# underdoc-wang/MPGCN

Measured on NVIDIA H100. Metric: OD-cells/sec (B*T*N^2), MPGCN hot path fwd+bwd, higher is better.
Workload: dtype f16

## Files before the change

mpgcn_b200/csrc/tc_engine.cuh:

```cuda
#pragma once

#include "common.cuh"
#include "wgmma.cuh"

#include <type_traits>

namespace mpgcn {
namespace tc {

enum AKind : int { A_MN128 = 0, A_K128 = 1, A_K64 = 2, A_MN64 = 3 };

struct OperandMap {
  int z_div, z_mod, z_mul;
  int seg_mod, seg_mul, seg_hi_mul;
  int k_seg;
};

struct Epilogue {
  void* out;
  __half* out16;
  long long sZ, sI, sR;
  int m_valid, r_valid;
  int out_f16;
  int relu;
  const float* bias;
  float alpha;
  const float* alpha_dev;
  float* absmax_out;
  const __half* corr_src;
  const float* corr_delta;
  long long cZ, cI, cR, cSeg;
  int corr_nseg;
};

struct alignas(64) GemmParams {
  CUtensorMap a_map;
  CUtensorMap b_map;
  OperandMap am, bm;
  int MT, NT, Z;
  int R;
  int kb_total, kb_per_seg;
  int split_k, kb_per_slice;
  int stages;
  int b_res_reps;
  int z_inner;
  Epilogue ep;
};

constexpr int kConsumerWGs = 2;
constexpr int kThreads1 = 128 * kConsumerWGs;
constexpr int kEpiRow = 40;
constexpr size_t kEpiBytes = (size_t)kConsumerWGs * 2 * 64 * kEpiRow * sizeof(float);

template <int AK, int BK>
struct Cfg {
  static constexpr int A_STAGE = (AK == A_MN128) ? BK * 256 : (AK == A_K128) ? 128 * 128 : (AK == A_K64) ? 128 * 64 * (BK / 32) : 4 * BK * 64;
  static constexpr bool A_MN = (AK == A_MN128) || (AK == A_MN64);
  static constexpr uint32_t A_KSTEP = (AK == A_MN128) ? 16 * 128 : (AK == A_MN64) ? 16 * 64 : 32;
  static constexpr uint32_t A_LBO = (AK == A_MN128) ? BK * 128 : (AK == A_MN64) ? BK * 64 : 16;
  static constexpr uint32_t A_SBO = (AK == A_MN128 || AK == A_K128) ? 1024 : 512;
  static constexpr uint32_t A_LAYOUT = (AK == A_MN128 || AK == A_K128) ? GMMA_SW128 : GMMA_SW64;
  static constexpr uint32_t B_KSTEP = 16 * 64;
  static constexpr uint32_t B_LBO = BK * 64;
  static constexpr uint32_t B_SBO = 512;
  static_assert(AK != A_K128 || BK == 64, "K-major SW128 rows hold exactly 64 halves");
  static_assert(AK != A_K64 || BK % 32 == 0, "K-major SW64 rows hold exactly 32 halves: BK counts whole planes");
  static constexpr uint32_t A_WG = (AK == A_MN128) ? BK * 128 : (AK == A_K128) ? 64 * 128 : (AK == A_K64) ? 64 * 64 : 2 * BK * 64;
  __host__ __device__ static constexpr uint32_t a_koff(int k) {
    return (AK == A_K64) ? (uint32_t)(k >> 1) * 8192u + (uint32_t)(k & 1) * 32u : (uint32_t)k * A_KSTEP;
  }
  static_assert(BK % 16 == 0, "wgmma K is 16 for fp16");
};

__host__ __device__ inline size_t smem_bytes(int a_stage, int R, int BK, int stages, int b_resident_tiles = 0) {
  const size_t b_stage = (size_t)R * BK * 64;
  return 1024  + (size_t)stages * a_stage + (size_t)(b_resident_tiles ? b_resident_tiles : stages) * b_stage + kEpiBytes +
         512 ;
}

#ifdef __CUDACC__
__device__ __forceinline__ void decode_tile(const GemmParams& p, int t, int& mt, int& nt, int& z) {
  if (p.z_inner > 1) {
    mt = t % p.MT;
    int rest = t / p.MT;
    const int zi = rest % p.z_inner;
    rest /= p.z_inner;
    nt = rest % p.NT;
    z = (rest / p.NT) * p.z_inner + zi;
  } else {
    mt = t % p.MT;
    const int rest = t / p.MT;
    nt = rest % p.NT;
    z = rest / p.NT;
  }
}

__device__ __forceinline__ void st_global_256(void* ptr, uint32_t a0, uint32_t a1, uint32_t a2, uint32_t a3, uint32_t a4, uint32_t a5,
                                              uint32_t a6, uint32_t a7) {
  uint4* d = reinterpret_cast<uint4*>(ptr);
  d[0] = make_uint4(a0, a1, a2, a3);
  d[1] = make_uint4(a4, a5, a6, a7);
}
__device__ __forceinline__ uint32_t pack_h2(float a, float b) { return f2h2_sat_bits(a, b); }

__device__ __forceinline__ void store_chunk(const Epilogue& ep, float alpha, const float* sbias, long long off,
                                            uint32_t (&acc)[32], float& amax) {
  float v[32];
#pragma unroll
  for (int c = 0; c < 32; ++c) {
    float x = __uint_as_float(acc[c]) * alpha;
    if (ep.bias) x += sbias[c];
    if (ep.relu) x = fmaxf(x, 0.f);
    v[c] = x;
  }
  if (ep.absmax_out) {
#pragma unroll
    for (int c = 0; c < 32; ++c) amax = fmaxf(amax, fabsf(v[c]));
  }
  if (ep.out_f16) {
    __half* dst = reinterpret_cast<__half*>(ep.out) + off;
#pragma unroll
    for (int q = 0; q < 2; ++q)
      st_global_256(dst + 16 * q, pack_h2(v[16 * q + 0], v[16 * q + 1]), pack_h2(v[16 * q + 2], v[16 * q + 3]),
                    pack_h2(v[16 * q + 4], v[16 * q + 5]), pack_h2(v[16 * q + 6], v[16 * q + 7]), pack_h2(v[16 * q + 8], v[16 * q + 9]),
                    pack_h2(v[16 * q + 10], v[16 * q + 11]), pack_h2(v[16 * q + 12], v[16 * q + 13]), pack_h2(v[16 * q + 14], v[16 * q + 15]));
  } else {
    float* dst = reinterpret_cast<float*>(ep.out) + off;
#pragma unroll
    for (int q = 0; q < 4; ++q)
      st_global_256(dst + 8 * q, __float_as_uint(v[8 * q + 0]), __float_as_uint(v[8 * q + 1]), __float_as_uint(v[8 * q + 2]),
                    __float_as_uint(v[8 * q + 3]), __float_as_uint(v[8 * q + 4]), __float_as_uint(v[8 * q + 5]),
                    __float_as_uint(v[8 * q + 6]), __float_as_uint(v[8 * q + 7]));
    if (ep.out16) {
      __half* d16 = ep.out16 + off;
#pragma unroll
      for (int q = 0; q < 2; ++q)
        st_global_256(d16 + 16 * q, pack_h2(v[16 * q + 0], v[16 * q + 1]), pack_h2(v[16 * q + 2], v[16 * q + 3]),
                      pack_h2(v[16 * q + 4], v[16 * q + 5]), pack_h2(v[16 * q + 6], v[16 * q + 7]), pack_h2(v[16 * q + 8], v[16 * q + 9]),
                      pack_h2(v[16 * q + 10], v[16 * q + 11]), pack_h2(v[16 * q + 12], v[16 * q + 13]), pack_h2(v[16 * q + 14], v[16 * q + 15]));
    }
  }
}

template <int AK, int BK>
__global__ void __launch_bounds__(kThreads1, 1) contract_kernel(const __grid_constant__ GemmParams p) {
  using C = Cfg<AK, BK>;
  constexpr int A_STAGE = C::A_STAGE;
  const int R = p.R;
  const int B_STAGE = R * BK * 64;
  const int S = p.stages;

  extern __shared__ uint8_t smem_raw[];
  uint8_t* smem = smem_raw + ((1024u - (smem_u32(smem_raw) & 1023u)) & 1023u);
  const int NRES = p.b_res_reps * p.kb_total;
  uint8_t* sA = smem;
  uint8_t* sB = sA + (size_t)S * A_STAGE;
  float* sEpi = reinterpret_cast<float*>(sB + (size_t)(NRES ? NRES : S) * B_STAGE);
  uint64_t* full = reinterpret_cast<uint64_t*>(reinterpret_cast<uint8_t*>(sEpi) + kEpiBytes);
  uint64_t* empty = full + S;
  uint64_t* bres_full = empty + S;
  float* sbias = reinterpret_cast<float*>(bres_full + 1);

  const int warp = threadIdx.x >> 5;
  const int lane = threadIdx.x & 31;

  if (threadIdx.x == 0) {
    tma_prefetch_desc(&p.a_map);
    tma_prefetch_desc(&p.b_map);
    for (int s = 0; s < S; ++s) {
      mbar_init(&full[s], 1);
      mbar_init(&empty[s], 4 * kConsumerWGs);
    }
    mbar_init(bres_full, 1);
    fence_barrier_init();
  }
  if (warp == 0) sbias[lane] = p.ep.bias ? p.ep.bias[lane] : 0.f;
  __syncthreads();

  const int num_tiles = p.MT * p.NT * p.Z;

  int p_t = blockIdx.x, p_kb = 0, p_kb1 = 0, p_kk = 0, p_sa_lo = 0, p_sa_hi = 0, p_sb_lo = 0, p_sb_hi = 0, p_zA0 = 0, p_zB0 = 0, p_mt = 0, p_nt = 0;
  int p_stage = 0;
  uint32_t p_phase = 0;
  auto p_start_tile = [&]() {
    int z;
    decode_tile(p, p_t, p_mt, p_nt, z);
    p_kb = p.split_k ? z * p.kb_per_slice : 0;
    p_kb1 = p.split_k ? min(p_kb + p.kb_per_slice, p.kb_total) : p.kb_total;
    p_zA0 = ((z / p.am.z_div) % p.am.z_mod) * p.am.z_mul;
    p_zB0 = ((z / p.bm.z_div) % p.bm.z_mod) * p.bm.z_mul;
    const int seg = p_kb / p.kb_per_seg;
    p_kk = p_kb - seg * p.kb_per_seg;
    p_sa_lo = seg % p.am.seg_mod; p_sa_hi = seg / p.am.seg_mod;
    p_sb_lo = seg % p.bm.seg_mod; p_sb_hi = seg / p.bm.seg_mod;
  };
  auto produce = [&]() {
    if (p_t >= num_tiles) return;
    mbar_wait_inline(&empty[p_stage], p_phase ^ 1u);
    mbar_arrive_expect_tx(&full[p_stage], (uint32_t)(A_STAGE + (NRES ? 0 : B_STAGE)));
    const int zA = p_zA0 + p_sa_lo * p.am.seg_mul + p_sa_hi * p.am.seg_hi_mul;
    const int zB = p_zB0 + p_sb_lo * p.bm.seg_mul + p_sb_hi * p.bm.seg_hi_mul;
    const int kA = p_kk * BK + p_sa_lo * p.am.k_seg;
    const int kB = p_kk * BK + p_sb_lo * p.bm.k_seg;
    uint8_t* a_dst = sA + (size_t)p_stage * A_STAGE;
    uint8_t* b_dst = sB + (size_t)p_stage * B_STAGE;
    if (AK == A_MN128) {
      tma_load_4d(a_dst, &p.a_map, &full[p_stage], p_mt * 128, kA, zA, 0);
      tma_load_4d(a_dst + BK * 128, &p.a_map, &full[p_stage], p_mt * 128 + 64, kA, zA, 0);
    } else if (AK == A_K128 || AK == A_K64) {
      tma_load_4d(a_dst, &p.a_map, &full[p_stage], kA, p_mt * 128, zA, 0);
    } else {
      tma_load_4d(a_dst, &p.a_map, &full[p_stage], 0, kA, p_mt * 4, zA);
    }
    if (!NRES)
      tma_load_4d(b_dst, &p.b_map, &full[p_stage], 0, kB, p_nt * R, zB);
    if (++p_stage == S) { p_stage = 0; p_phase ^= 1u; }
    if (++p_kk == p.kb_per_seg) {
      p_kk = 0;
      if (++p_sa_lo == p.am.seg_mod) { p_sa_lo = 0; ++p_sa_hi; }
      if (++p_sb_lo == p.bm.seg_mod) { p_sb_lo = 0; ++p_sb_hi; }
    }
    if (++p_kb == p_kb1) {
      p_t += gridDim.x;
      if (p_t < num_tiles) p_start_tile();
    }
  };
  if (threadIdx.x == 0 && (int)blockIdx.x < num_tiles) {
    if (NRES) {
      mbar_arrive_expect_tx(bres_full, (uint32_t)(NRES * B_STAGE));
      for (int sg = 0; sg < NRES; ++sg) {
        const int lo = sg % p.bm.seg_mod, hi = sg / p.bm.seg_mod;
        tma_load_4d(sB + (size_t)sg * B_STAGE, &p.b_map, bres_full, 0, lo * p.bm.k_seg, 0, lo * p.bm.seg_mul + hi * p.bm.seg_hi_mul);
      }
    }
    p_start_tile();
    for (int s = 0; s < S; ++s) produce();
  }
  __syncwarp();

  {
    const int wg = warp >> 2;
    const int tw = threadIdx.x & 127;
    const int wq = warp & 3, g = lane >> 2, q = lane & 3;
    const float alpha = p.ep.alpha_dev ? p.ep.alpha * __ldg(p.ep.alpha_dev) : p.ep.alpha;
    const uint64_t a_hi = gmma_desc_hi(C::A_SBO, C::A_LAYOUT);
    const uint64_t b_hi = gmma_desc_hi(C::B_SBO, GMMA_SW64);
    float* stg = sEpi + (size_t)wg * 2 * 64 * kEpiRow;
    float amax = 0.f;
    float acc[128];
    int stage = 0;
    uint32_t phase = 0;
    if (NRES && (int)blockIdx.x < num_tiles) mbar_wait_inline(bres_full, 0);
    for (int t = blockIdx.x; t < num_tiles; t += gridDim.x) {
      int mt, nt, z;
      decode_tile(p, t, mt, nt, z);
      const int kb0 = p.split_k ? z * p.kb_per_slice : 0;
      const int kb1 = p.split_k ? min(kb0 + p.kb_per_slice, p.kb_total) : p.kb_total;
      int prev = -1;
      for (int kb = kb0; kb < kb1; ++kb) {
        mbar_wait_inline(&full[stage], phase);
        const uint32_t a_addr = smem_u32(sA + (size_t)stage * A_STAGE) + C::A_WG * (uint32_t)wg;
        const int reps = NRES ? p.b_res_reps : 1;
        wgmma_fence();
        for (int rep = 0; rep < reps; ++rep) {
          const uint32_t b_addr = smem_u32(sB + (size_t)(NRES ? rep * p.kb_total + kb : stage) * B_STAGE);
          const int first = (kb == kb0 && rep == 0) ? 1 : 0;
          auto kblock = [&](auto width) {
            constexpr int RW = decltype(width)::value;
#pragma unroll
            for (int k = 0; k < BK / 16; ++k) {
              const uint64_t ad = gmma_desc(a_hi, a_addr + C::a_koff(k), C::A_LBO);
              const uint64_t bd = gmma_desc(b_hi, b_addr + k * C::B_KSTEP, C::B_LBO);
              wgmma_n<RW, C::A_MN ? 1 : 0, 1>(acc, ad, bd, (first && k == 0) ? 0 : 1);
            }
          };
          switch (R) {
            case 1: kblock(std::integral_constant<int, 1>()); break;
            case 2: kblock(std::integral_constant<int, 2>()); break;
            case 3: kblock(std::integral_constant<int, 3>()); break;
            case 4: kblock(std::integral_constant<int, 4>()); break;
            case 5: kblock(std::integral_constant<int, 5>()); break;
            case 6: kblock(std::integral_constant<int, 6>()); break;
            case 7: kblock(std::integral_constant<int, 7>()); break;
            default: kblock(std::integral_constant<int, 8>()); break;
          }
        }
        wgmma_commit();
        wgmma_wait<1>();
        if (prev >= 0) {
          __syncwarp();
          if (lane == 0) mbar_arrive(&empty[prev]);
          if (threadIdx.x == 0) produce();
          __syncwarp();
        }
        prev = stage;
        if (++stage == S) { stage = 0; phase ^= 1u; }
      }
      wgmma_wait<0>();
      if (prev >= 0) {
        __syncwarp();
        if (lane == 0) mbar_arrive(&empty[prev]);
        if (threadIdx.x == 0) produce();
        __syncwarp();
      }
      const int half = tw >> 6, rr = tw & 63;
      const int i = mt * 128 + wg * 64 + rr;
      const long long base = (long long)z * p.ep.sZ + (long long)i * p.ep.sI;
      float dl[8];
      long long cbase = 0;
      bool any_corr = false;
      if (p.ep.corr_src != nullptr) {
        const int zA = ((z / p.am.z_div) % p.am.z_mod) * p.am.z_mul;
        const int zB = ((z / p.bm.z_div) % p.bm.z_mod) * p.bm.z_mul;
        cbase = (long long)zB * p.ep.cZ + (long long)i * p.ep.cI;
#pragma unroll
        for (int sgi = 0; sgi < 8; ++sgi) {
          dl[sgi] = (sgi < p.ep.corr_nseg && i < p.ep.m_valid)
                        ? __ldg(p.ep.corr_delta + ((long long)zA * p.ep.corr_nseg + sgi) * p.ep.m_valid + i) : 0.f;
          any_corr |= (dl[sgi] != 0.f);
        }
      }
#pragma unroll
      for (int j0 = 0; j0 < 8; j0 += 2) {
        if (j0 < R) {
#pragma unroll
          for (int s = 0; s < 2; ++s) {
            if (j0 + s < R) {
#pragma unroll
              for (int jj = 0; jj < 4; ++jj)
#pragma unroll
                for (int h = 0; h < 2; ++h)
                  *reinterpret_cast<float2*>(stg + (s * 64 + 16 * wq + g + 8 * h) * kEpiRow + 8 * jj + 2 * q) =
                      make_float2(acc[16 * (j0 + s) + 4 * jj + 2 * h], acc[16 * (j0 + s) + 4 * jj + 2 * h + 1]);
            }
          }
          named_bar_sync(1 + wg, 128);
          const int j = j0 + half;
          const int r = nt * R + j;
          if (j < R && i < p.ep.m_valid && r < p.ep.r_valid) {
            uint32_t regs[32];
#pragma unroll
            for (int c = 0; c < 32; c += 4) {
              const float4 v = *reinterpret_cast<const float4*>(stg + (half * 64 + rr) * kEpiRow + c);
              regs[c] = __float_as_uint(v.x); regs[c + 1] = __float_as_uint(v.y);
              regs[c + 2] = __float_as_uint(v.z); regs[c + 3] = __float_as_uint(v.w);
            }
            if (any_corr) {
#pragma unroll
              for (int sgi = 0; sgi < 8; ++sgi) {
                if (sgi < p.ep.corr_nseg && dl[sgi] != 0.f) {
                  const uint4* src = reinterpret_cast<const uint4*>(p.ep.corr_src + cbase + (long long)sgi * p.ep.cSeg + (long long)r * p.ep.cR);
#pragma unroll
                  for (int qq = 0; qq < 4; ++qq) {
                    const uint4 v = __ldg(src + qq);
                    const __half2* h2 = reinterpret_cast<const __half2*>(&v);
#pragma unroll
                    for (int e = 0; e < 4; ++e) {
                      const float2 f = __half22float2(h2[e]);
                      regs[8 * qq + 2 * e] = __float_as_uint(fmaf(dl[sgi], f.x, __uint_as_float(regs[8 * qq + 2 * e])));
                      regs[8 * qq + 2 * e + 1] = __float_as_uint(fmaf(dl[sgi], f.y, __uint_as_float(regs[8 * qq + 2 * e + 1])));
                    }
                  }
                }
              }
            }
            store_chunk(p.ep, alpha, sbias, base + (long long)r * p.ep.sR, regs, amax);
          }
          named_bar_sync(1 + wg, 128);
        }
      }
    }
    if (p.ep.absmax_out) {
      for (int o = 16; o > 0; o >>= 1) amax = fmaxf(amax, __shfl_xor_sync(0xffffffffu, amax, o));
      if (lane == 0) atomicMax(reinterpret_cast<unsigned int*>(p.ep.absmax_out), __float_as_uint(amax));
    }
  }
}
#endif

int launch_contract(int ak, int bk, GemmParams& p, cudaStream_t stream);

}
}
```

Baseline: 392.9 million.

## Add dedicated TMA producer warpgroup with register reallocation to GEMM engine

Adds a third warpgroup that acts only as the TMA producer, giving up registers via setmaxnreg while the two consumer warpgroups raise their register budget. Consumers no longer issue produce() calls inline after each k-block, so loads for later tiles proceed without waiting on consumer progress. The correction-delta values are now re-read from global memory inside the epilogue instead of being held in an 8-entry register array, which lowers register pressure at the cost of extra loads. Waits switch to plain spin loops, and the launch now uses 384 threads per block, which lowers occupancy headroom.

Measured after the change: 398.8 million (median of 6 runs). 1.01x the previous value.

```diff
diff --git a/mpgcn_b200/csrc/tc_engine.cuh b/mpgcn_b200/csrc/tc_engine.cuh
--- a/mpgcn_b200/csrc/tc_engine.cuh
+++ b/mpgcn_b200/csrc/tc_engine.cuh
@@ -48,7 +48,9 @@
 };
 
 constexpr int kConsumerWGs = 2;
-constexpr int kThreads1 = 128 * kConsumerWGs;
+constexpr int kThreads1 = 128 * (1 + kConsumerWGs);
+constexpr int kProducerRegs = 40;
+constexpr int kConsumerRegs = 232;
 constexpr int kEpiRow = 40;
 constexpr size_t kEpiBytes = (size_t)kConsumerWGs * 2 * 64 * kEpiRow * sizeof(float);
 
@@ -102,6 +104,16 @@
   d[1] = make_uint4(a4, a5, a6, a7);
 }
 __device__ __forceinline__ uint32_t pack_h2(float a, float b) { return f2h2_sat_bits(a, b); }
+
+template <int REGS>
+__device__ __forceinline__ void setmaxnreg_dec() { asm volatile("setmaxnreg.dec.sync.aligned.u32 %0;" ::"n"(REGS)); }
+template <int REGS>
+__device__ __forceinline__ void setmaxnreg_inc() { asm volatile("setmaxnreg.inc.sync.aligned.u32 %0;" ::"n"(REGS)); }
+
+__device__ __forceinline__ void mbar_wait_spin(uint64_t* bar, uint32_t parity) {
+  while (!mbar_try_wait(bar, parity)) {
+  }
+}
 
 __device__ __forceinline__ void store_chunk(const Epilogue& ep, float alpha, const float* sbias, long long off,
                                             uint32_t (&acc)[32], float& amax) {
@@ -225,21 +237,29 @@
       if (p_t < num_tiles) p_start_tile();
     }
   };
-  if (threadIdx.x == 0 && (int)blockIdx.x < num_tiles) {
-    if (NRES) {
-      mbar_arrive_expect_tx(bres_full, (uint32_t)(NRES * B_STAGE));
-      for (int sg = 0; sg < NRES; ++sg) {
-        const int lo = sg % p.bm.seg_mod, hi = sg / p.bm.seg_mod;
-        tma_load_4d(sB + (size_t)sg * B_STAGE, &p.b_map, bres_full, 0, lo * p.bm.k_seg, 0, lo * p.bm.seg_mul + hi * p.bm.seg_hi_mul);
-      }
-    }
-    p_start_tile();
-    for (int s = 0; s < S; ++s) produce();
-  }
-  __syncwarp();
-
+  if (__shfl_sync(0xffffffffu, (int)threadIdx.x >> 7, 0) == 0) {
+    setmaxnreg_dec<kProducerRegs>();
+    if (threadIdx.x == 0 && (int)blockIdx.x < num_tiles) {
+      if (NRES) {
+        mbar_arrive_expect_tx(bres_full, (uint32_t)(NRES * B_STAGE));
+        for (int sg = 0; sg < NRES; ++sg) {
+          const int lo = sg % p.bm.seg_mod, hi = sg / p.bm.seg_mod;
+          tma_load_4d(sB + (size_t)sg * B_STAGE, &p.b_map, bres_full, 0, lo * p.bm.k_seg, 0, lo * p.bm.seg_mul + hi * p.bm.seg_hi_mul);
+        }
+      }
+      p_start_tile();
+      while (p_t < num_tiles) produce();
+      for (int s = 0; s < S; ++s) {
+        mbar_wait_inline(&empty[p_stage], p_phase ^ 1u);
+        if (++p_stage == S) { p_stage = 0; p_phase ^= 1u; }
+      }
+    }
+    return;
+  }
+
+  setmaxnreg_inc<kConsumerRegs>();
   {
-    const int wg = warp >> 2;
+    const int wg = (warp >> 2) - 1;
     const int tw = threadIdx.x & 127;
     const int wq = warp & 3, g = lane >> 2, q = lane & 3;
     const float alpha = p.ep.alpha_dev ? p.ep.alpha * __ldg(p.ep.alpha_dev) : p.ep.alpha;
@@ -250,7 +270,7 @@
     float acc[128];
     int stage = 0;
     uint32_t phase = 0;
-    if (NRES && (int)blockIdx.x < num_tiles) mbar_wait_inline(bres_full, 0);
+    if (NRES && (int)blockIdx.x < num_tiles) mbar_wait_spin(bres_full, 0);
     for (int t = blockIdx.x; t < num_tiles; t += gridDim.x) {
       int mt, nt, z;
       decode_tile(p, t, mt, nt, z);
@@ -258,7 +278,7 @@
       const int kb1 = p.split_k ? min(kb0 + p.kb_per_slice, p.kb_total) : p.kb_total;
       int prev = -1;
       for (int kb = kb0; kb < kb1; ++kb) {
-        mbar_wait_inline(&full[stage], phase);
+        mbar_wait_spin(&full[stage], phase);
         const uint32_t a_addr = smem_u32(sA + (size_t)stage * A_STAGE) + C::A_WG * (uint32_t)wg;
         const int reps = NRES ? p.b_res_reps : 1;
         wgmma_fence();
@@ -290,8 +310,6 @@
         if (prev >= 0) {
           __syncwarp();
           if (lane == 0) mbar_arrive(&empty[prev]);
-          if (threadIdx.x == 0) produce();
-          __syncwarp();
         }
         prev = stage;
         if (++stage == S) { stage = 0; phase ^= 1u; }
@@ -300,25 +318,20 @@
       if (prev >= 0) {
         __syncwarp();
         if (lane == 0) mbar_arrive(&empty[prev]);
-        if (threadIdx.x == 0) produce();
-        __syncwarp();
       }
       const int half = tw >> 6, rr = tw & 63;
       const int i = mt * 128 + wg * 64 + rr;
       const long long base = (long long)z * p.ep.sZ + (long long)i * p.ep.sI;
-      float dl[8];
       long long cbase = 0;
+      const float* dl = nullptr;
       bool any_corr = false;
-      if (p.ep.corr_src != nullptr) {
+      if (p.ep.corr_src != nullptr && i < p.ep.m_valid) {
         const int zA = ((z / p.am.z_div) % p.am.z_mod) * p.am.z_mul;
         const int zB = ((z / p.bm.z_div) % p.bm.z_mod) * p.bm.z_mul;
         cbase = (long long)zB * p.ep.cZ + (long long)i * p.ep.cI;
-#pragma unroll
-        for (int sgi = 0; sgi < 8; ++sgi) {
-          dl[sgi] = (sgi < p.ep.corr_nseg && i < p.ep.m_valid)
-                        ? __ldg(p.ep.corr_delta + ((long long)zA * p.ep.corr_nseg + sgi) * p.ep.m_valid + i) : 0.f;
-          any_corr |= (dl[sgi] != 0.f);
-        }
+        dl = p.ep.corr_delta + (long long)zA * p.ep.corr_nseg * p.ep.m_valid + i;
+#pragma unroll 1
+        for (int sgi = 0; sgi < p.ep.corr_nseg; ++sgi) any_corr |= (__ldg(dl + (long long)sgi * p.ep.m_valid) != 0.f);
       }
 #pragma unroll
       for (int j0 = 0; j0 < 8; j0 += 2) {
@@ -346,9 +359,10 @@
               regs[c + 2] = __float_as_uint(v.z); regs[c + 3] = __float_as_uint(v.w);
             }
             if (any_corr) {
-#pragma unroll
-              for (int sgi = 0; sgi < 8; ++sgi) {
-                if (sgi < p.ep.corr_nseg && dl[sgi] != 0.f) {
+#pragma unroll 1
+              for (int sgi = 0; sgi < p.ep.corr_nseg; ++sgi) {
+                const float d = __ldg(dl + (long long)sgi * p.ep.m_valid);
+                if (d != 0.f) {
                   const uint4* src = reinterpret_cast<const uint4*>(p.ep.corr_src + cbase + (long long)sgi * p.ep.cSeg + (long long)r * p.ep.cR);
 #pragma unroll
                   for (int qq = 0; qq < 4; ++qq) {
@@ -357,8 +371,8 @@
 #pragma unroll
                     for (int e = 0; e < 4; ++e) {
                       const float2 f = __half22float2(h2[e]);
-                      regs[8 * qq + 2 * e] = __float_as_uint(fmaf(dl[sgi], f.x, __uint_as_float(regs[8 * qq + 2 * e])));
-                      regs[8 * qq + 2 * e + 1] = __float_as_uint(fmaf(dl[sgi], f.y, __uint_as_float(regs[8 * qq + 2 * e + 1])));
+                      regs[8 * qq + 2 * e] = __float_as_uint(fmaf(d, f.x, __uint_as_float(regs[8 * qq + 2 * e])));
+                      regs[8 * qq + 2 * e + 1] = __float_as_uint(fmaf(d, f.y, __uint_as_float(regs[8 * qq + 2 * e + 1])));
                     }
                   }
                 }
```
